# leeyevi/MV3D_TF

Measured on AMD Instinct MI355X. Metric: KITTI-shape frames/sec (RPN+3-view ROI-pool+NMS) at 1/2/4/8 MI355X, higher is better.
Workload: dtype f32; 1 GPU; BASELINE configs[2] path-only: batch 2, 3 views; proposal_layer_3d TRAIN cfg (23104 BEV anchors, pre/post-NMS 12000/2000, NMS 0.7) + anchor_target + proposal_target (256 sampled ROIs in batch 0) + FV ROIs + RoiPool 7x7 fwd+bwd on BEV 76x76x512 / RGB 46x155x512 / FV 8x64x512; peaky scores; driven by the library's own mv3d_train_path (submit -> counts to the host -> numpy-global-RNG draws on the hel; batch_per_gpu=2, ring_batches=16, streams=8, launch=path, hipgraph=False, parallelism=frames/1, pmc_signature=train/b2/r256/peaky/pair-tiles-planned

## Files before the change

include/mv3d_hip.h:

```cpp
#ifndef MV3D_HIP_H
#define MV3D_HIP_H
#include <stddef.h>
#include <stdint.h>
#ifdef __cplusplus
extern "C" {
#endif

typedef enum {
    MV3D_OK = 0,
    MV3D_ERR_INVALID_ARG = 1,
    MV3D_ERR_WORKSPACE = 2,
    MV3D_ERR_HIP = 3,
    MV3D_ERR_ZERO_DIVISION = 4
} mv3d_status;

int mv3d_version(void);
const char *mv3d_status_string(int status);


size_t mv3d_nms_workspace_bytes(int max_boxes);
int mv3d_nms_device(const float *dets_dev, int n, double thresh, int max_keep,
                    int32_t *keep_dev, int32_t *num_keep_dev, int32_t *status_dev,
                    void *workspace, size_t workspace_bytes, void *stream);

// ... 112 lines not shown
int mv3d_anchor_target_stage2(int H, int W, const mv3d_anchor_target_params *p,
                              const int32_t *disable_fg_dev, int n_dis_fg,
                              const int32_t *disable_bg1_dev, int n_dis_bg1,
                              const int32_t *disable_bg2_dev, int n_dis_bg2,
                              float *labels_dev, float *anchors_dev, float *anchors_3d_dev,
                              int32_t *n_anchors_dev, int anchors_cap,
                              void *workspace, size_t workspace_bytes, void *stream);

int mv3d_anchor_target_stage1_batch(int batch, int H, int W, const float *im_info_dev, const float *const *gt_bv_dev,
                                    const float *const *gt_3d_dev, const int *G, const mv3d_anchor_target_params *p,
                                    float *labels_dev, float *targets_dev, int32_t *const *counts_dev,
                                    uint8_t *const *fg_hi_dev, void *const *workspace, size_t workspace_bytes, void *stream);
int mv3d_anchor_target_stage1_batch_masked(int batch, int H, int W, const float *im_info_dev, const float *const *gt_bv_dev,
                                           const float *const *gt_3d_dev, const int *G, const mv3d_anchor_target_params *p,
                                           const uint8_t *const *anchor_mask_dev, float *labels_dev, float *targets_dev,
                                           int32_t *const *counts_dev, uint8_t *const *fg_hi_dev, void *const *workspace,
                                           size_t workspace_bytes, void *stream);
int mv3d_anchor_target_stage2_batch(int batch, int H, int W, const mv3d_anchor_target_params *p,
                                    const int32_t *const *disable_fg_dev, const int *n_dis_fg,
                                    const int32_t *const *disable_bg1_dev, const int *n_dis_bg1,
                                    const int32_t *const *disable_bg2_dev, const int *n_dis_bg2, float *labels_dev,
                                    float *anchors_dev, float *anchors_3d_dev, int32_t *n_anchors_dev, int anchors_cap,
                                    void *const *workspace, size_t workspace_bytes, void *stream);

typedef struct {
    int32_t num_classes;
    int32_t frame_index;
    double fg_thresh;
    double bg_thresh_hi;
    double bg_thresh_lo;
} mv3d_proposal_target_params;

size_t mv3d_proposal_target_workspace_bytes(int num_rois, int G);
int mv3d_proposal_target_stage1(const float *rois_bv_dev, const float *rois_3d_dev, int num_rois,
                                const float *gt_bv_dev, const float *gt_3d_dev, int G,
                                const mv3d_proposal_target_params *p, int32_t *counts_dev,
                                void *workspace, size_t workspace_bytes, void *stream);
int mv3d_proposal_target_stage2(const float *rois_bv_dev, const float *rois_3d_dev, int num_rois,
                                const float *gt_bv_dev, const float *gt_3d_dev,
                                const float *gt_corners_dev, int G, const float *calib_dev,
                                const mv3d_proposal_target_params *p,
                                const int32_t *fg_pick_dev, int n_fg, const int32_t *bg_pick_dev, int n_bg,
                                float *rois_bv_out, float *rois_img_out, int32_t *labels_out,
                                float *bbox_targets_out, float *rois_3d_out,
                                void *workspace, size_t workspace_bytes, void *stream);

// ... 13 lines not shown
                                           const int *num_rois_cap, const int32_t *const *num_rois_dev,
                                           const float *const *gt_bv_dev, const float *const *gt_3d_dev, const int *G,
                                           const mv3d_proposal_target_params *params, int32_t *const *counts_dev,
                                           void *const *workspace, const size_t *workspace_bytes, void *stream);
int mv3d_proposal_target_stage2_batch_devn(int batch, const float *const *rois_bv_dev, const float *const *rois_3d_dev,
                                           const int *num_rois_cap, const int32_t *const *num_rois_dev,
                                           const float *const *gt_bv_dev, const float *const *gt_3d_dev,
                                           const float *const *gt_corners_dev, const int *G, const float *const *calib_dev,
                                           const mv3d_proposal_target_params *params, const int32_t *const *fg_pick_dev,
                                           const int *n_fg, const int32_t *const *bg_pick_dev, const int *n_bg,
                                           float *const *rois_bv_out, float *const *rois_img_out, int32_t *const *labels_out,
                                           float *const *bbox_targets_out, float *const *rois_3d_out, float *const *rois_fv_out,
                                           void *const *workspace, const size_t *workspace_bytes, void *stream);

int mv3d_point_cloud_2_top(const float *points_dev, int num_points, float *top_dev, void *stream);

int mv3d_point_cloud_2_top_shape(double res, double zres, double side_lo, double side_hi, double fwd_lo, double fwd_hi,
                                 double height_lo, double height_hi, int *dims);
int mv3d_point_cloud_2_top_ranges(const float *points_dev, int num_points, double res, double zres, double side_lo, double side_hi,
                                  double fwd_lo, double fwd_hi, double height_lo, double height_hi, float *top_dev,
                                  int *status_dev, void *stream);

int mv3d_legacy_permutation(void *mt19937_state, int32_t n, int32_t *out);
typedef struct {
    int32_t n_fg, n_bg, n_low;
    int32_t pt_n_fg, pt_n_bg;
    int32_t reserved0;
    const uint8_t *fg_alive;
} mv3d_draw_frame;
typedef struct {
    int32_t rpn_batchsize;
    int32_t rpn_num_fg;
    int32_t rois_per_image;
    int32_t roi_fg_max;
} mv3d_draw_params;
int mv3d_draw_training_subsamples(void *mt19937_state, int batch, const mv3d_draw_frame *frames, const mv3d_draw_params *par,
                                  int32_t *lists, size_t lists_cap, int32_t *sizes, int32_t *scratch, size_t scratch_cap);

typedef struct {
    int32_t batch, H, W, num_classes;
    int32_t proposal_cap;
    int32_t anchor_cap;
    int32_t roi_cap;
    int32_t max_gt;
    mv3d_proposal_params proposal;
    mv3d_anchor_target_params anchor;
    mv3d_proposal_target_params target;
    mv3d_draw_params draw;
} mv3d_train_path_config;
typedef struct {
    float *blob_bv, *blob_img, *blob_3d;
    int32_t *num_proposals;
    void *proposal_ws; size_t proposal_ws_bytes;
    float *rpn_labels, *rpn_targets;
    float *anchors, *anchors_3d;
    int32_t *n_anchors;
    uint8_t *report; size_t report_row;
    int32_t *pt_counts;
    void *anchor_ws; size_t anchor_ws_bytes;
    void *target_ws; size_t target_ws_bytes;
// ... 237 lines not shown
```

mv3d_tf_amd/_lib.py:

```python
import ctypes as C
import os

import torch

_HERE = os.path.dirname(os.path.abspath(__file__))
LIB_PATH = os.path.join(_HERE, "libmv3d_hip.so")

OK, ERR_INVALID_ARG, ERR_WORKSPACE, ERR_HIP, ERR_ZERO_DIVISION = 0, 1, 2, 3, 4


class ProposalParams(C.Structure):
    _fields_ = [("feat_stride", C.c_int32), ("pre_nms_topN", C.c_int32), ("post_nms_topN", C.c_int32),
                ("img_height", C.c_int32), ("img_width", C.c_int32), ("img_padding", C.c_int32),
                ("nms_strict_gt", C.c_int32), ("reserved0", C.c_int32), ("nms_thresh", C.c_double), ("min_size", C.c_double)]


class DetectPostParams(C.Structure):
    _fields_ = [("num_classes", C.c_int32), ("rows_per_frame", C.c_int32), ("max_per_image", C.c_int32),
                ("nms_strict_gt", C.c_int32), ("score_thresh", C.c_float), ("reserved0", C.c_int32), ("nms_thresh", C.c_double)]


class AnchorTargetParams(C.Structure):
    _fields_ = [("feat_stride", C.c_int32), ("clobber_positives", C.c_int32),
                ("negative_overlap", C.c_double), ("positive_overlap", C.c_double)]
# ... 108 lines not shown
    "mv3d_proposal_3d_workspace_bytes": (C.c_size_t, [C.c_int, C.c_int, C.c_int, C.POINTER(ProposalParams)]),
    "mv3d_proposal_3d": (C.c_int, [_P, _P, C.c_int, C.c_int, C.c_int, _P, _P, C.POINTER(ProposalParams),
                                   _P, _P, _P, _P, _P, _P, C.c_size_t, _P]),
    "mv3d_proposal_3d_masked": (C.c_int, [_P, _P, C.c_int, C.c_int, C.c_int, _P, _P, C.POINTER(ProposalParams),
                                          _P, _P, _P, _P, _P, _P, _P, C.c_size_t, _P]),
    "mv3d_anchor_occupancy_workspace_bytes": (C.c_size_t, [C.c_int, C.c_int, C.c_int]),
    "mv3d_anchor_occupancy": (C.c_int, [_P, C.c_int, C.c_int, C.c_int, C.c_int, C.c_int, C.c_int, C.c_int, C.c_int, _P, _P, _P,
                                        C.c_size_t, _P]),
    "mv3d_roi_pool_forward": (C.c_int, [_P, C.c_float, C.c_int, C.c_int, C.c_int, C.c_int, C.c_int, C.c_int,
                                        C.c_int, _P, _P, _P, _P]),
    "mv3d_roi_pool_backward": (C.c_int, [_P, C.c_float, C.c_int, C.c_int, C.c_int, C.c_int, C.c_int, C.c_int,
                                         C.c_int, _P, _P, _P, _P]),
    "mv3d_anchor_target_workspace_bytes": (C.c_size_t, [C.c_int, C.c_int, C.c_int]),
    "mv3d_anchor_target_stage1": (C.c_int, [C.c_int, C.c_int, _P, _P, _P, C.c_int, C.POINTER(AnchorTargetParams),
                                            _P, _P, _P, _P, _P, C.c_size_t, _P]),
    "mv3d_anchor_target_stage2": (C.c_int, [C.c_int, C.c_int, C.POINTER(AnchorTargetParams), _P, C.c_int, _P,
                                            C.c_int, _P, C.c_int, _P, _P, _P, _P, C.c_int, _P, C.c_size_t, _P]),
    "mv3d_anchor_target_stage1_batch": (C.c_int, [C.c_int, C.c_int, C.c_int, _P, _P, _P, _P, C.POINTER(AnchorTargetParams), _P, _P, _P, _P,
                                                  _P, C.c_size_t, _P]),
    "mv3d_anchor_target_stage1_batch_masked": (C.c_int, [C.c_int, C.c_int, C.c_int, _P, _P, _P, _P, C.POINTER(AnchorTargetParams), _P, _P,
                                                         _P, _P, _P, _P, C.c_size_t, _P]),
    "mv3d_anchor_target_stage2_batch": (C.c_int, [C.c_int, C.c_int, C.c_int, C.POINTER(AnchorTargetParams), _P, _P, _P, _P, _P, _P, _P,
                                                  _P, _P, _P, C.c_int, _P, C.c_size_t, _P]),
    "mv3d_proposal_target_stage1_batch": (C.c_int, [C.c_int, _P, _P, _P, _P, _P, _P, _P, _P, _P, _P, _P]),
    "mv3d_proposal_target_stage2_batch": (C.c_int, [C.c_int, _P, _P, _P, _P, _P, _P, _P, _P, _P, _P, _P, _P, _P, _P, _P, _P, _P, _P, _P,
                                                    _P, _P, _P]),
    "mv3d_proposal_target_stage1_batch_devn": (C.c_int, [C.c_int, _P, _P, _P, _P, _P, _P, _P, _P, _P, _P, _P, _P]),
    "mv3d_proposal_target_stage2_batch_devn": (C.c_int, [C.c_int, _P, _P, _P, _P, _P, _P, _P, _P, _P, _P, _P, _P, _P, _P, _P, _P, _P, _P,
                                                         _P, _P, _P, _P, _P]),
    "mv3d_proposal_target_workspace_bytes": (C.c_size_t, [C.c_int, C.c_int]),
    "mv3d_proposal_target_stage1": (C.c_int, [_P, _P, C.c_int, _P, _P, C.c_int, C.POINTER(ProposalTargetParams), _P, _P,
                                              C.c_size_t, _P]),
    "mv3d_proposal_target_stage2": (C.c_int, [_P, _P, C.c_int, _P, _P, _P, C.c_int, _P, C.POINTER(ProposalTargetParams),
                                              _P, C.c_int, _P, C.c_int, _P, _P, _P, _P, _P, _P, C.c_size_t, _P]),
    "mv3d_point_cloud_2_top": (C.c_int, [_P, C.c_int, _P, _P]),
    "mv3d_point_cloud_2_top_shape": (C.c_int, [C.c_double] * 8 + [_P]),
    "mv3d_point_cloud_2_top_ranges": (C.c_int, [_P, C.c_int] + [C.c_double] * 8 + [_P, _P, _P]),
    "mv3d_box_detect_tail": (C.c_int, [_P, _P, C.c_int, C.c_int, _P, _P, _P, _P, _P]),
    "mv3d_detect_post_workspace_bytes": (C.c_size_t, [C.c_int, C.POINTER(DetectPostParams)]),
    "mv3d_detect_post": (C.c_int, [_P, _P, _P, _P, _P, C.c_int, C.POINTER(DetectPostParams), _P, _P, _P, _P, _P, _P, _P, C.c_size_t,
                                   _P]),
    "mv3d_detect_post_oriented_workspace_bytes": (C.c_size_t, [C.c_int, C.POINTER(DetectPostParams)]),
    "mv3d_detect_post_oriented": (C.c_int, [_P, _P, _P, _P, _P, C.c_int, C.POINTER(DetectPostParams), C.c_int, _P, _P, _P, _P, _P, _P,
                                            _P, C.c_size_t, _P]),
    "mv3d_loss_workspace_bytes": (C.c_size_t, [C.c_int]),
    "mv3d_rpn_loss": (C.c_int, [_P, _P, _P, _P, C.c_int, C.c_float, _P, _P, _P, _P, C.c_size_t, _P]),
    "mv3d_rcnn_loss": (C.c_int, [_P, _P, _P, _P, C.c_int, C.c_int, C.c_int, C.c_float, _P, _P, _P, _P, C.c_size_t, _P]),
    "mv3d_roi_pool_forward_views": (C.c_int, [C.c_int, C.POINTER(RoiView), C.c_int, C.c_int, _P]),
    "mv3d_roi_pool_forward_views_cold": (C.c_int, [C.c_int, C.POINTER(RoiView), C.c_int, C.c_int, _P]),
    "mv3d_roi_pool_forward_views_half": (C.c_int, [C.c_int, C.POINTER(RoiView), C.c_int, C.c_int, C.c_int, C.c_int, _P]),
    "mv3d_roi_pool_backward_workspace_bytes": (C.c_size_t, [C.c_int, C.POINTER(RoiGradView), C.c_int, C.c_int]),
    "mv3d_roi_pool_backward_views": (C.c_int, [C.c_int, C.POINTER(RoiGradView), C.c_int, C.c_int, _P, C.c_size_t, _P]),
    "mv3d_roi_pool_pair_workspace_bytes": (C.c_size_t, [C.c_int, C.POINTER(RoiGradView), C.c_int, C.c_int]),
    "mv3d_roi_pool_forward_views_pair": (C.c_int, [C.c_int, C.POINTER(RoiView), C.c_int, C.c_int, C.c_int, _P]),
    "mv3d_roi_pool_backward_views_pair": (C.c_int, [C.c_int, C.POINTER(RoiGradView), C.c_int, C.c_int, _P, C.c_size_t, _P]),
    "mv3d_roi_pool_argmax_decode": (C.c_int, [C.c_int, C.POINTER(RoiView), C.c_int, C.c_int, C.POINTER(C.c_void_p), _P]),
    "mv3d_ROIPoolForwardLaucher": (C.c_int, [_P, C.c_float, C.c_int, C.c_int, C.c_int, C.c_int, C.c_int, C.c_int, _P, _P, _P, _P]),
    "mv3d_ROIPoolBackwardLaucher": (C.c_int, [_P, C.c_float, C.c_int, C.c_int, C.c_int, C.c_int, C.c_int, C.c_int, C.c_int, _P, _P, _P, _P]),
    "mv3d_rois_3d_to_fv": (C.c_int, [_P, C.c_int, _P, _P]),
    "mv3d_legacy_permutation": (C.c_int, [_P, C.c_int32, _P]),
    "mv3d_draw_training_subsamples": (C.c_int, [_P, C.c_int, C.POINTER(DrawFrame), C.POINTER(DrawParams), _P, C.c_size_t, _P, _P,
                                                C.c_size_t]),
    "mv3d_train_path_create": (C.c_int, [C.POINTER(TrainPathConfig), C.c_int, C.POINTER(TrainPathSlot), C.c_int, C.POINTER(C.c_void_p)]),
    "mv3d_train_path_configure": (C.c_int, [_P, C.POINTER(TrainPathConfig)]),
    "mv3d_train_path_submit": (C.c_int, [_P, C.c_int, _P, _P, _P, _P, _P, _P, _P, _P, _P, _P]),
    "mv3d_train_path_submit_masked": (C.c_int, [_P, C.c_int, _P, _P, _P, _P, _P, _P, _P, _P, _P, _P, _P]),
    "mv3d_train_path_finish": (C.c_int, [_P, C.c_int, _P, _P, _P]),
    "mv3d_train_path_host_seconds": (C.c_int, [_P, C.POINTER(C.c_double), C.POINTER(C.c_double)]),
    "mv3d_train_path_destroy": (None, [_P]),
    "mv3d_gt_encode": (C.c_int, [_P, _P, C.c_int, _P, _P, _P, _P, _P, _P, _P]),
    "mv3d_conv3x3_f16": (C.c_int, [_P, _P, _P, _P, C.c_int, C.c_int, C.c_int, C.c_int, C.c_int, C.c_int, C.c_int, C.c_int, _P]),
    "mv3d_conv3x3_f32": (C.c_int, [_P, _P, _P, _P, C.c_int, C.c_int, C.c_int, C.c_int, C.c_int, C.c_int, C.c_int, _P]),
    "mv3d_maxpool2x2_f32": (C.c_int, [_P, _P, C.c_int, C.c_int, C.c_int, C.c_int, _P]),
    "mv3d_frame_nhwc_f32": (C.c_int, [_P, _P, C.c_int, C.c_int, C.c_int, C.c_int, C.c_int, _P]),
    "mv3d_conv3x3_bf16": (C.c_int, [_P, _P, _P, _P, C.c_int, C.c_int, C.c_int, C.c_int, C.c_int, C.c_int, C.c_int, C.c_int, _P]),
    "mv3d_maxpool2x2_bf16": (C.c_int, [_P, _P, C.c_int, C.c_int, C.c_int, C.c_int, _P]),
    "mv3d_frame_nhwc_bf16": (C.c_int, [_P, _P, C.c_int, C.c_int, C.c_int, C.c_int, C.c_int, _P]),
    "mv3d_conv3x3_wgrad_workspace_bytes": (C.c_size_t, [C.c_int, C.c_int, C.c_int, C.c_int, C.c_int]),
    "mv3d_conv3x3_wgrad_bf16": (C.c_int, [_P, _P, _P, _P, C.c_int, C.c_int, C.c_int, C.c_int, C.c_int, C.c_int, _P, C.c_size_t, _P]),
    "mv3d_conv3x3_wgrad_f32_workspace_bytes": (C.c_size_t, [C.c_int, C.c_int, C.c_int, C.c_int, C.c_int]),
    "mv3d_conv3x3_wgrad_f32": (C.c_int, [_P, _P, _P, _P, C.c_int, C.c_int, C.c_int, C.c_int, C.c_int, C.c_int, _P, C.c_size_t, _P]),
    "mv3d_conv3x3_pack_bf16": (C.c_int, [_P, _P, _P, C.c_int, C.c_int, C.c_int, _P]),
    "mv3d_conv3x3_gated_bf16": (C.c_int, [_P, _P, _P, _P, _P, C.c_int, C.c_int, C.c_int, C.c_int, C.c_int, _P]),
    "mv3d_maxpool2x2_bwd_f32": (C.c_int, [_P, _P, _P, C.c_int, C.c_int, C.c_int, C.c_int, _P]),
    "mv3d_maxpool2x2_bwd_bf16": (C.c_int, [_P, _P, _P, C.c_int, C.c_int, C.c_int, C.c_int, _P]),
# ... 70 lines not shown
```

mv3d_tf_amd/csrc/anchor_target.hip:

```cpp
#include <math.h>
#include "geometry.h"

__device__ __forceinline__ double mv3d_log(double x)
{
    if (x != x || x < 0) return NAN;
    if (x == 0) return -INFINITY;
    if (isinf(x)) return x;
    int k;
    double m = frexp(x, &k);
    if (m < 0.70710678118654752440) { m *= 2.0; k -= 1; }
    const double s = (m - 1.0) / (m + 1.0);
    const double z = s * s;
    double p = 1.0 / 39;
#pragma unroll
    for (int d = 37; d >= 1; d -= 2) p = fma(p, z, 1.0 / d);
    const double LN2_HI = 6.93147180369123816490e-01, LN2_LO = 1.90821492927058770002e-10;
    const double lm = 2.0 * s * p;
    return fma((double)k, LN2_HI, fma((double)k, LN2_LO, lm));
}

struct AtDev {
    int H, W, N, G, stride, clobber;
    double neg_ov, pos_ov;
    const float *im_info, *gt_bv, *gt_3d;
// ... 126 lines not shown
            f[0] = inside; f[1] = inside && (lab == 1.0f); f[2] = inside && (lab == 0.0f); f[3] = inside && (mx < neg_ov);
        },
        [&](int k, int pos, int n) {
            if (k == 1) { L.fg[pos] = n; fg_hi[pos] = (max_ov[n] >= neg_ov) ? 1 : 0; }
            else if (k == 2) L.bg[pos] = n;
            else if (k == 3) L.low[pos] = n;
        },
        F.agg1, tot);
    if (blockIdx.x == gridDim.x - 1 && threadIdx.x == 0) {
        int32_t *counts = F.counts;
        counts[0] = tot[0]; counts[1] = tot[1]; counts[2] = tot[2]; counts[3] = tot[3];
        counts[4] = counts[5] = counts[6] = counts[7] = 0;
    }
}

__global__ __launch_bounds__(256) void at_disable_all_kernel(AtBatch bt)
{
    const AtFrame &F = bt.f[blockIdx.y];
    const int n1 = F.n_dis_fg, n2 = F.n_dis_bg1, n3 = F.n_dis_bg2;
    for (int t = blockIdx.x * blockDim.x + threadIdx.x; t < n1 + n2 + n3; t += gridDim.x * blockDim.x) {
        if (t < n1) F.d.labels[F.lists.fg[F.dis_fg[t]]] = -1.0f;
        else if (t < n1 + n2) F.d.labels[F.lists.bg[F.dis_bg1[t - n1]]] = -1.0f;
        else F.d.argmax[F.lists.low[F.dis_bg2[t - n1 - n2]]] = -1;
    }
}

__global__ __launch_bounds__(256) void at_emit_relabel_kernel(AtBatch bt)
{
    const AtFrame &F = bt.f[blockIdx.y];
    const AtDev &d = F.d;
    float *anchors = F.anchors, *anchors_3d = F.anchors_3d;
    const int cap = bt.cap;
    int tot[1];
    mv3d_grid_compact<1>(
        d.N,
        [&](int n, bool f[1]) { f[0] = anchors && (d.max_ov[n] >= 0.0) && (d.labels[n] != -1.0f); },
        [&](int, int r, int n) {
            if (r >= cap) return;
            int x1, y1, x2, y2;
            grid_anchor(n, d.W, d.stride, x1, y1, x2, y2);
            float *A = anchors + 5 * (long long)r, *B = anchors_3d + 7 * (long long)r;
            A[0] = 0.0f; A[1] = (float)x1; A[2] = (float)y1; A[3] = (float)x2; A[4] = (float)y2;
            B[0] = 0.0f;
            anchor_to_lidar(x1, y1, x2, y2, B + 1);
        },
        F.agg2, tot);
// ... 85 lines not shown
    hipLaunchKernelGGL(at_compact_kernel, dim3(L.ncwg, batch), dim3(256), 0, s, bt);
    return mv3d_launch_status();
}

extern "C" int mv3d_anchor_target_stage1_batch(int batch, int H, int W, const float *im_info_dev, const float *const *gt_bv_dev,
                                               const float *const *gt_3d_dev, const int *G, const mv3d_anchor_target_params *p,
                                               float *labels_dev, float *targets_dev, int32_t *const *counts_dev,
                                               uint8_t *const *fg_hi_dev, void *const *workspace, size_t workspace_bytes,
                                               void *stream)
{
    return mv3d_anchor_target_stage1_batch_masked(batch, H, W, im_info_dev, gt_bv_dev, gt_3d_dev, G, p, nullptr, labels_dev, targets_dev,
                                                  counts_dev, fg_hi_dev, workspace, workspace_bytes, stream);
}

extern "C" int mv3d_anchor_target_stage1(int H, int W, const float *im_info_dev, const float *gt_bv_dev,
                                         const float *gt_3d_dev, int G, const mv3d_anchor_target_params *p,
                                         float *labels_dev, float *targets_dev, int32_t *counts_dev, uint8_t *fg_hi_dev,
                                         void *workspace, size_t workspace_bytes, void *stream)
{
    return mv3d_anchor_target_stage1_batch(1, H, W, im_info_dev, &gt_bv_dev, &gt_3d_dev, &G, p, labels_dev, targets_dev,
                                           &counts_dev, &fg_hi_dev, &workspace, workspace_bytes, stream);
}

extern "C" int mv3d_anchor_target_stage2_batch(int batch, int H, int W, const mv3d_anchor_target_params *p,
                                               const int32_t *const *disable_fg_dev, const int *n_dis_fg,
                                               const int32_t *const *disable_bg1_dev, const int *n_dis_bg1,
                                               const int32_t *const *disable_bg2_dev, const int *n_dis_bg2, float *labels_dev,
                                               float *anchors_dev, float *anchors_3d_dev, int32_t *n_anchors_dev,
                                               int anchors_cap, void *const *workspace, size_t workspace_bytes, void *stream)
{
    if (batch <= 0 || batch > AT_MAX_BATCH || !p || !labels_dev || !workspace || !n_dis_fg || !n_dis_bg1 || !n_dis_bg2 ||
        !disable_fg_dev || !disable_bg1_dev || !disable_bg2_dev)
        return MV3D_ERR_INVALID_ARG;
    AtLayout L;
    if (!at_layout(H, W, 0, L)) return MV3D_ERR_INVALID_ARG;
    const bool emit = anchors_dev && anchors_3d_dev && n_anchors_dev;
    AtBatch bt = {};
    bt.cap = anchors_cap;
    int most = 0;
    for (int b = 0; b < batch; ++b) {
        if (n_dis_fg[b] < 0 || n_dis_bg1[b] < 0 || n_dis_bg2[b] < 0) return MV3D_ERR_INVALID_ARG;
        if ((n_dis_fg[b] && !disable_fg_dev[b]) || (n_dis_bg1[b] && !disable_bg1_dev[b]) || (n_dis_bg2[b] && !disable_bg2_dev[b]))
            return MV3D_ERR_INVALID_ARG;
        if (!workspace[b] || workspace_bytes < L.total || ((uintptr_t)workspace[b] % MV3D_ALIGN)) return MV3D_ERR_WORKSPACE;
        AtFrame &F = bt.f[b];
        at_frame(F, L, H, W, 0, p, (char *)workspace[b]);
        F.d.im_info = nullptr; F.d.gt_bv = nullptr; F.d.gt_3d = nullptr; F.d.mask = nullptr; F.d.targets = nullptr;
        F.d.labels = labels_dev + (size_t)b * L.N;
        F.dis_fg = disable_fg_dev[b]; F.dis_bg1 = disable_bg1_dev[b]; F.dis_bg2 = disable_bg2_dev[b];
        F.n_dis_fg = n_dis_fg[b]; F.n_dis_bg1 = n_dis_bg1[b]; F.n_dis_bg2 = n_dis_bg2[b];
        F.anchors = emit ? anchors_dev + (size_t)b * anchors_cap * 5 : nullptr;
        F.anchors_3d = emit ? anchors_3d_dev + (size_t)b * anchors_cap * 7 : nullptr;
        F.n_anchors = emit ? n_anchors_dev + b : nullptr;
        const int n = n_dis_fg[b] + n_dis_bg1[b] + n_dis_bg2[b];
        if (n > most) most = n;
    }
    hipStream_t s = (hipStream_t)stream;
    if (most > 0) hipLaunchKernelGGL(at_disable_all_kernel, dim3((most + 255) / 256, batch), dim3(256), 0, s, bt);
    hipLaunchKernelGGL(at_emit_relabel_kernel, dim3(L.ncwg, batch), dim3(256), 0, s, bt);
    return mv3d_launch_status();
}

extern "C" int mv3d_anchor_target_stage2(int H, int W, const mv3d_anchor_target_params *p,
                                         const int32_t *disable_fg_dev, int n_dis_fg, const int32_t *disable_bg1_dev,
                                         int n_dis_bg1, const int32_t *disable_bg2_dev, int n_dis_bg2, float *labels_dev,
                                         float *anchors_dev, float *anchors_3d_dev, int32_t *n_anchors_dev,
                                         int anchors_cap, void *workspace, size_t workspace_bytes, void *stream)
{
    return mv3d_anchor_target_stage2_batch(1, H, W, p, &disable_fg_dev, &n_dis_fg, &disable_bg1_dev, &n_dis_bg1, &disable_bg2_dev,
                                           &n_dis_bg2, labels_dev, anchors_dev, anchors_3d_dev, n_anchors_dev, anchors_cap,
                                           &workspace, workspace_bytes, stream);
}
```

mv3d_tf_amd/csrc/legacy_rng.hip:

```cpp
#include <stdint.h>
#include <string.h>
#include "../../include/mv3d_hip.h"

namespace {

constexpr int MT_N = 624, MT_M = 397;
struct MtState { uint32_t key[MT_N]; int pos; };

inline void mt_gen(MtState *s)
{
    uint32_t *k = s->key;
    int i;
    for (i = 0; i < MT_N - MT_M; ++i) {
        const uint32_t y = (k[i] & 0x80000000u) | (k[i + 1] & 0x7fffffffu);
        k[i] = k[i + MT_M] ^ (y >> 1) ^ ((y & 1u) ? 0x9908b0dfu : 0u);
    }
    for (; i < MT_N - 1; ++i) {
        const uint32_t y = (k[i] & 0x80000000u) | (k[i + 1] & 0x7fffffffu);
        k[i] = k[i + (MT_M - MT_N)] ^ (y >> 1) ^ ((y & 1u) ? 0x9908b0dfu : 0u);
    }
    const uint32_t y = (k[MT_N - 1] & 0x80000000u) | (k[0] & 0x7fffffffu);
    k[MT_N - 1] = k[MT_M - 1] ^ (y >> 1) ^ ((y & 1u) ? 0x9908b0dfu : 0u);
    s->pos = 0;
}
// ... 25 lines not shown
                for (int k = pos; k < MT_N; ++k) {
                    uint32_t y = s->key[k];
                    y ^= (y >> 11);
                    y ^= (y << 7) & 0x9d2c5680u;
                    y ^= (y << 15) & 0xefc60000u;
                    y ^= (y >> 18);
                    t[k] = y;
                }
                t_lo = pos;
            }
            while (pos < MT_N && i > lo) {
                const uint32_t j = t[pos++] & mask;
                const bool ok = j <= (uint32_t)i;
                const uint32_t jj = ok ? j : (uint32_t)i;
                const int32_t a = x[i], b = x[jj];
                x[i] = b; x[jj] = a;
                i -= ok ? 1 : 0;
            }
        }
    }
    s->pos = pos;
}

}

extern "C" int mv3d_legacy_permutation(void *mt19937_state, int32_t n, int32_t *out)
{
    if (!mt19937_state || n < 0 || (n > 0 && !out)) return MV3D_ERR_INVALID_ARG;
    MtState *s = (MtState *)mt19937_state;
    if (s->pos < 0 || s->pos > MT_N) return MV3D_ERR_INVALID_ARG;
    permutation(s, n, out);
    return MV3D_OK;
}

extern "C" int mv3d_draw_training_subsamples(void *mt19937_state, int batch, const mv3d_draw_frame *frames,
                                             const mv3d_draw_params *par, int32_t *lists, size_t lists_cap, int32_t *sizes,
                                             int32_t *scratch, size_t scratch_cap)
{
    if (!mt19937_state || batch <= 0 || !frames || !par || !lists || !sizes || !scratch) return MV3D_ERR_INVALID_ARG;
    MtState *s = (MtState *)mt19937_state;
    if (s->pos < 0 || s->pos > MT_N) return MV3D_ERR_INVALID_ARG;
    size_t o = 0;
    auto emit = [&](int32_t n, int32_t take, bool draw, int32_t *size_out) -> bool {
        *size_out = 0;
        if (!draw) return true;
        if (n < 0 || (size_t)n > scratch_cap || take < 0 || take > n || o + (size_t)take > lists_cap) return false;
// ... 15 lines not shown
        const int32_t num_fg = par->rpn_num_fg;
        const int32_t *dis_fg = lists + o;
        if (!emit(f.n_fg, f.n_fg - num_fg, f.n_fg > num_fg, &sz[0])) return MV3D_ERR_WORKSPACE;
        const int32_t num_bg = par->rpn_batchsize - (f.n_fg < num_fg ? f.n_fg : num_fg);
        if (!emit(f.n_bg, f.n_bg - num_bg, f.n_bg > num_bg, &sz[1])) return MV3D_ERR_WORKSPACE;
        int32_t n_pos = 0;
        if (f.n_fg > 0) {
            if ((size_t)f.n_fg > scratch_cap) return MV3D_ERR_WORKSPACE;
            uint8_t *alive = (uint8_t *)scratch;
            for (int32_t i = 0; i < f.n_fg; ++i) alive[i] = f.fg_alive[i] ? 1 : 0;
            for (int32_t i = 0; i < sz[0]; ++i) alive[dis_fg[i]] = 0;
            for (int32_t i = 0; i < f.n_fg; ++i) n_pos += alive[i];
        }
        const int32_t num_bg2 = par->rpn_batchsize - n_pos;
        if (!emit(f.n_low, f.n_low - num_bg2, f.n_low > num_bg2, &sz[2])) return MV3D_ERR_WORKSPACE;
        const int32_t fg_n = par->roi_fg_max < f.pt_n_fg ? par->roi_fg_max : f.pt_n_fg;
        if (!emit(f.pt_n_fg, fg_n, f.pt_n_fg > 0, &sz[3])) return MV3D_ERR_WORKSPACE;
        const int32_t bg_room = par->rois_per_image - fg_n;
        const int32_t bg_n = bg_room < f.pt_n_bg ? bg_room : f.pt_n_bg;
        if (!emit(f.pt_n_bg, bg_n < 0 ? 0 : bg_n, f.pt_n_bg > 0, &sz[4])) return MV3D_ERR_WORKSPACE;
    }
    return MV3D_OK;
}
```

mv3d_tf_amd/csrc/train_stream.hip:

```cpp
#include <hip/hip_runtime.h>
#include <chrono>
#include <condition_variable>
#include <deque>
#include <mutex>
#include <new>
#include <thread>
#include <vector>
#include "common.h"
#include "../../include/mv3d_hip.h"

#define TP_MAX_BATCH 16

namespace {

enum SlotState { TP_IDLE = 0, TP_SUBMITTED = 1, TP_STAGED = 2 };

struct Slot {
    mv3d_train_path_slot buf;
    hipEvent_t ev = nullptr;
    int state = TP_IDLE, rc = MV3D_OK;
    hipStream_t stream = nullptr;
    void *mt = nullptr;
    const float *calib = nullptr;
    const float *gt_bv[TP_MAX_BATCH], *gt_3d[TP_MAX_BATCH], *gt_c[TP_MAX_BATCH];
    int G[TP_MAX_BATCH];
    int32_t sizes[5 * TP_MAX_BATCH], rows[TP_MAX_BATCH];
    std::vector<uint8_t> spill[TP_MAX_BATCH];
    float *p_bv[TP_MAX_BATCH], *p_3d[TP_MAX_BATCH];
    int32_t *p_num[TP_MAX_BATCH], *p_cnt[TP_MAX_BATCH], *a_cnt[TP_MAX_BATCH];
    uint8_t *a_fgh[TP_MAX_BATCH];
    void *a_ws[TP_MAX_BATCH], *p_ws[TP_MAX_BATCH];
    int p_cap[TP_MAX_BATCH];
    size_t p_wsz[TP_MAX_BATCH];
    uint8_t *dv_report = nullptr;
    int32_t *dv_pt_counts = nullptr, *dv_num_proposals = nullptr;
};

static bool tp_force_copies()
{
#ifdef MV3D_TUNING
    return getenv("MV3D_TRAIN_PATH_COPIES") != nullptr;
#else
    return false;
#endif
}

__global__ __launch_bounds__(256) void tp_report_kernel(const uint8_t *__restrict__ report, size_t report_row, uint8_t *__restrict__ h_report,
                                                        size_t h_row, int B, const int32_t *__restrict__ pt_counts, int32_t *__restrict__ h_pt,
                                                        const int32_t *__restrict__ nump, int32_t *__restrict__ h_nump)
{
    const size_t v = h_row / 16;
    for (size_t i = threadIdx.x; i < (size_t)B * v; i += 256) {
        const size_t b = i / v, j = i - b * v;
        reinterpret_cast<uint4 *>(h_report + b * h_row)[j] = reinterpret_cast<const uint4 *>(report + b * report_row)[j];
    }
    for (int i = threadIdx.x; i < 4 * B; i += 256) h_pt[i] = pt_counts[i];
    for (int i = threadIdx.x; i < 2 * B; i += 256) h_nump[i] = nump[i];
}
// ... 75 lines not shown
    const int B = c.batch, H = c.H, W = c.W;
    const auto t0 = std::chrono::steady_clock::now();
    TP_HIP(hipEventSynchronize(s.ev));
    const auto t1 = std::chrono::steady_clock::now();
    for (int b = 0; b < B; ++b)
        if (u.h_num_proposals[B + b] & MV3D_FLAG_ZERO_DIVISION) return MV3D_ERR_ZERO_DIVISION;
    mv3d_draw_frame fr[TP_MAX_BATCH];
    for (int b = 0; b < B; ++b) {
        const uint8_t *head = u.h_report + (size_t)b * u.h_report_row;
        const int32_t *cnt = (const int32_t *)head;
        fr[b].n_fg = cnt[1]; fr[b].n_bg = cnt[2]; fr[b].n_low = cnt[3];
        fr[b].pt_n_fg = u.h_pt_counts[4 * b + 1]; fr[b].pt_n_bg = u.h_pt_counts[4 * b + 2];
        fr[b].reserved0 = 0;
        if (cnt[1] < 0 || (size_t)cnt[1] > (size_t)4 * H * W) return MV3D_ERR_INVALID_ARG;
        if (32 + (size_t)cnt[1] <= u.h_report_row) {
            fr[b].fg_alive = head + 32;
        } else {
            s.spill[b].resize((size_t)cnt[1]);
            TP_HIP(hipMemcpyAsync(s.spill[b].data(), s.a_fgh[b], (size_t)cnt[1], hipMemcpyDeviceToHost, s.stream));
            TP_HIP(hipStreamSynchronize(s.stream));
            fr[b].fg_alive = s.spill[b].data();
        }
    }
    int rc = mv3d_draw_training_subsamples(s.mt, B, fr, &c.draw, u.h_lists, u.lists_cap, s.sizes, u.h_scratch, u.scratch_cap);
    const auto t2 = std::chrono::steady_clock::now();
    {
        std::lock_guard<std::mutex> g(tp->m);
        tp->t_wait += std::chrono::duration<double>(t1 - t0).count();
        tp->t_draw += std::chrono::duration<double>(t2 - t1).count();
    }
    if (rc != MV3D_OK) return rc;
    size_t off[5 * TP_MAX_BATCH + 1];
    off[0] = 0;
    for (int k = 0; k < 5 * B; ++k) off[k + 1] = off[k] + (size_t)s.sizes[k];
    const int32_t *const lists = u.lists;
    if (off[5 * B]) TP_HIP(hipMemcpyAsync(u.lists, u.h_lists, off[5 * B] * sizeof(int32_t), hipMemcpyHostToDevice, s.stream));
    const int32_t *lst[5][TP_MAX_BATCH];
    int cnt[5][TP_MAX_BATCH];
    for (int b = 0; b < B; ++b)
        for (int k = 0; k < 5; ++k) {
            cnt[k][b] = s.sizes[5 * b + k];
            lst[k][b] = cnt[k][b] ? lists + off[5 * b + k] : nullptr;
        }
    rc = mv3d_anchor_target_stage2_batch(B, H, W, &c.anchor, lst[0], cnt[0], lst[1], cnt[1], lst[2], cnt[2], u.rpn_labels, u.anchors,
                                         u.anchors_3d, u.n_anchors, c.anchor_cap, s.a_ws, u.anchor_ws_bytes, s.stream);
    if (rc != MV3D_OK) return rc;
    float *o_bev[TP_MAX_BATCH], *o_rgb[TP_MAX_BATCH], *o_fv[TP_MAX_BATCH], *o_3d[TP_MAX_BATCH], *o_tg[TP_MAX_BATCH];
    int32_t *o_lab[TP_MAX_BATCH];
    const float *cal[TP_MAX_BATCH];
    size_t row = 0;
    for (int b = 0; b < B; ++b) {
        const int S = cnt[3][b] + cnt[4][b];
        s.rows[b] = S;
        if (row + (size_t)S > (size_t)B * c.roi_cap) return MV3D_ERR_WORKSPACE;
        o_bev[b] = S ? u.rois_bev + row * 5 : nullptr;
        o_rgb[b] = S ? u.rois_rgb + row * 5 : nullptr;
        o_fv[b] = (S && u.rois_fv) ? u.rois_fv + row * 5 : nullptr;
        o_3d[b] = S ? u.rois_3d + row * 7 : nullptr;
        o_lab[b] = S ? u.labels + row : nullptr;
        o_tg[b] = S ? u.bbox_targets + row * 24 * c.num_classes : nullptr;
        cal[b] = s.calib + (size_t)b * 48;
        row += (size_t)S;
    }
    return mv3d_proposal_target_stage2_batch_devn(B, s.p_bv, s.p_3d, s.p_cap, s.p_num, s.gt_bv, s.gt_3d, s.gt_c, s.G, cal, tp->tpar, lst[3],
                                                  cnt[3], lst[4], cnt[4], o_bev, o_rgb, o_lab, o_tg, o_3d, u.rois_fv ? o_fv : nullptr, s.p_ws,
                                                  s.p_wsz, s.stream);
}

// ... 40 lines not shown
    mv3d_train_path *tp = new (std::nothrow) mv3d_train_path();
    if (!tp) return MV3D_ERR_HIP;
    set_params(tp, *config);
    tp->depth = depth;
    if (hipGetDevice(&tp->device) != hipSuccess) { delete tp; return MV3D_ERR_HIP; }
    try {
        tp->slots.resize((size_t)depth);
    } catch (...) {
        delete tp;
        return MV3D_ERR_HIP;
    }
    for (int k = 0; k < depth; ++k) {
        Slot &s = tp->slots[k];
        s.buf = slots[k];
        slot_tables(tp->cfg, s);
        {
            void *d0 = nullptr, *d1 = nullptr, *d2 = nullptr;
            const bool mapped = hipHostGetDevicePointer(&d0, s.buf.h_report, 0) == hipSuccess && hipHostGetDevicePointer(&d1, s.buf.h_pt_counts, 0) == hipSuccess &&
                                hipHostGetDevicePointer(&d2, s.buf.h_num_proposals, 0) == hipSuccess && d0 && d1 && d2;
            (void)hipGetLastError();
            if (mapped && s.buf.h_report_row % 16 == 0 && (uintptr_t)d0 % 16 == 0 && (uintptr_t)s.buf.report % 16 == 0 && !tp_force_copies()) {
                s.dv_report = (uint8_t *)d0; s.dv_pt_counts = (int32_t *)d1; s.dv_num_proposals = (int32_t *)d2;
            }
        }
        if (hipEventCreateWithFlags(&s.ev, hipEventDisableTiming | hipEventBlockingSync) != hipSuccess) {
            for (int j = 0; j < k; ++j) (void)hipEventDestroy(tp->slots[j].ev);
            delete tp;
            return MV3D_ERR_HIP;
        }
    }
    tp->threaded = helper_thread != 0;
    if (tp->threaded) {
        try {
            tp->helper = std::thread(helper_main, tp);
        } catch (...) {
            for (Slot &s : tp->slots) (void)hipEventDestroy(s.ev);
            delete tp;
            return MV3D_ERR_HIP;
        }
    }
    *out = tp;
    return MV3D_OK;
}

extern "C" int mv3d_train_path_configure(mv3d_train_path *tp, const mv3d_train_path_config *c)
{
// ... 134 lines not shown
```

Measured before the change: 16670 frames/s.

## Draw only kept tail of RNG permutations and pass keep-bitmasks to anchor disable

Host-side subsampling now computes only the last k entries of the legacy MT19937 permutation. It uses a sparse swap map and an SSE block-skip over the rejection-sampled prefix, so it no longer builds the full n-element shuffle for large candidate sets. Those entries are encoded as per-frame keep bitmasks instead of explicit disable index lists. A new disable kernel reads the bitmasks. The lists buffer is read through a mapped host pointer when available, which skips the H2D copy. This adds complex RNG-equivalence logic that must reproduce numpy's stream exactly, and zero-copy reads from pinned host memory over the bus.

```diff
diff --git a/include/mv3d_hip.h b/include/mv3d_hip.h
--- a/include/mv3d_hip.h
+++ b/include/mv3d_hip.h
@@ -158,6 +158,12 @@
                                     const int32_t *const *disable_bg2_dev, const int *n_dis_bg2, float *labels_dev,
                                     float *anchors_dev, float *anchors_3d_dev, int32_t *n_anchors_dev, int anchors_cap,
                                     void *const *workspace, size_t workspace_bytes, void *stream);
+int mv3d_anchor_target_stage2_batch_kept(int batch, int H, int W, const mv3d_anchor_target_params *p,
+                                         const int32_t *const *keep_fg_dev, const int *n_fg,
+                                         const int32_t *const *keep_bg1_dev, const int *n_bg,
+                                         const int32_t *const *keep_bg2_dev, const int *n_low, float *labels_dev,
+                                         float *anchors_dev, float *anchors_3d_dev, int32_t *n_anchors_dev, int anchors_cap,
+                                         void *const *workspace, size_t workspace_bytes, void *stream);
 
 typedef struct {
     int32_t num_classes;
@@ -217,6 +223,7 @@
                                   int *status_dev, void *stream);
 
 int mv3d_legacy_permutation(void *mt19937_state, int32_t n, int32_t *out);
+int mv3d_legacy_permutation_tail(void *mt19937_state, int32_t n, int32_t k, int32_t *out);
 typedef struct {
     int32_t n_fg, n_bg, n_low;
     int32_t pt_n_fg, pt_n_bg;
@@ -231,6 +238,8 @@
 } mv3d_draw_params;
 int mv3d_draw_training_subsamples(void *mt19937_state, int batch, const mv3d_draw_frame *frames, const mv3d_draw_params *par,
                                   int32_t *lists, size_t lists_cap, int32_t *sizes, int32_t *scratch, size_t scratch_cap);
+int mv3d_draw_training_subsamples_kept(void *mt19937_state, int batch, const mv3d_draw_frame *frames, const mv3d_draw_params *par,
+                                       int32_t *lists, size_t lists_cap, int32_t *sizes, int32_t *scratch, size_t scratch_cap);
 
 typedef struct {
     int32_t batch, H, W, num_classes;
diff --git a/mv3d_tf_amd/_lib.py b/mv3d_tf_amd/_lib.py
--- a/mv3d_tf_amd/_lib.py
+++ b/mv3d_tf_amd/_lib.py
@@ -154,6 +154,8 @@
                                                          _P, _P, _P, _P, C.c_size_t, _P]),
     "mv3d_anchor_target_stage2_batch": (C.c_int, [C.c_int, C.c_int, C.c_int, C.POINTER(AnchorTargetParams), _P, _P, _P, _P, _P, _P, _P,
                                                   _P, _P, _P, C.c_int, _P, C.c_size_t, _P]),
+    "mv3d_anchor_target_stage2_batch_kept": (C.c_int, [C.c_int, C.c_int, C.c_int, C.POINTER(AnchorTargetParams), _P, _P, _P, _P, _P, _P,
+                                                       _P, _P, _P, _P, C.c_int, _P, C.c_size_t, _P]),
     "mv3d_proposal_target_stage1_batch": (C.c_int, [C.c_int, _P, _P, _P, _P, _P, _P, _P, _P, _P, _P, _P]),
     "mv3d_proposal_target_stage2_batch": (C.c_int, [C.c_int, _P, _P, _P, _P, _P, _P, _P, _P, _P, _P, _P, _P, _P, _P, _P, _P, _P, _P, _P,
                                                     _P, _P, _P]),
@@ -193,6 +195,9 @@
     "mv3d_legacy_permutation": (C.c_int, [_P, C.c_int32, _P]),
     "mv3d_draw_training_subsamples": (C.c_int, [_P, C.c_int, C.POINTER(DrawFrame), C.POINTER(DrawParams), _P, C.c_size_t, _P, _P,
                                                 C.c_size_t]),
+    "mv3d_legacy_permutation_tail": (C.c_int, [_P, C.c_int32, C.c_int32, _P]),
+    "mv3d_draw_training_subsamples_kept": (C.c_int, [_P, C.c_int, C.POINTER(DrawFrame), C.POINTER(DrawParams), _P, C.c_size_t, _P, _P,
+                                                     C.c_size_t]),
     "mv3d_train_path_create": (C.c_int, [C.POINTER(TrainPathConfig), C.c_int, C.POINTER(TrainPathSlot), C.c_int, C.POINTER(C.c_void_p)]),
     "mv3d_train_path_configure": (C.c_int, [_P, C.POINTER(TrainPathConfig)]),
     "mv3d_train_path_submit": (C.c_int, [_P, C.c_int, _P, _P, _P, _P, _P, _P, _P, _P, _P, _P]),
diff --git a/mv3d_tf_amd/csrc/anchor_target.hip b/mv3d_tf_amd/csrc/anchor_target.hip
--- a/mv3d_tf_amd/csrc/anchor_target.hip
+++ b/mv3d_tf_amd/csrc/anchor_target.hip
@@ -172,6 +172,27 @@
         if (t < n1) F.d.labels[F.lists.fg[F.dis_fg[t]]] = -1.0f;
         else if (t < n1 + n2) F.d.labels[F.lists.bg[F.dis_bg1[t - n1]]] = -1.0f;
         else F.d.argmax[F.lists.low[F.dis_bg2[t - n1 - n2]]] = -1;
+    }
+}
+
+__global__ __launch_bounds__(256) void at_disable_kept_kernel(AtBatch bt)
+{
+    const AtFrame &F = bt.f[blockIdx.y];
+    const int n1 = F.n_dis_fg, n2 = F.n_dis_bg1, n3 = F.n_dis_bg2;
+    const unsigned N = (unsigned)F.d.N;
+    for (int t = blockIdx.x * blockDim.x + threadIdx.x; t < n1 + n2 + n3; t += gridDim.x * blockDim.x) {
+        if (t < n1) {
+            const unsigned a = (unsigned)F.lists.fg[t];
+            if (!((F.dis_fg[t >> 5] >> (t & 31)) & 1) && a < N) F.d.labels[a] = -1.0f;
+        } else if (t < n1 + n2) {
+            const int u = t - n1;
+            const unsigned a = (unsigned)F.lists.bg[u];
+            if (!((F.dis_bg1[u >> 5] >> (u & 31)) & 1) && a < N) F.d.labels[a] = -1.0f;
+        } else {
+            const int u = t - n1 - n2;
+            const unsigned a = (unsigned)F.lists.low[u];
+            if (!((F.dis_bg2[u >> 5] >> (u & 31)) & 1) && a < N) F.d.argmax[a] = -1;
+        }
     }
 }
 
@@ -303,12 +324,11 @@
                                            &counts_dev, &fg_hi_dev, &workspace, workspace_bytes, stream);
 }
 
-extern "C" int mv3d_anchor_target_stage2_batch(int batch, int H, int W, const mv3d_anchor_target_params *p,
-                                               const int32_t *const *disable_fg_dev, const int *n_dis_fg,
-                                               const int32_t *const *disable_bg1_dev, const int *n_dis_bg1,
-                                               const int32_t *const *disable_bg2_dev, const int *n_dis_bg2, float *labels_dev,
-                                               float *anchors_dev, float *anchors_3d_dev, int32_t *n_anchors_dev,
-                                               int anchors_cap, void *const *workspace, size_t workspace_bytes, void *stream)
+static int at_stage2(bool kept, int batch, int H, int W, const mv3d_anchor_target_params *p, const int32_t *const *disable_fg_dev,
+                     const int *n_dis_fg, const int32_t *const *disable_bg1_dev, const int *n_dis_bg1,
+                     const int32_t *const *disable_bg2_dev, const int *n_dis_bg2, float *labels_dev, float *anchors_dev,
+                     float *anchors_3d_dev, int32_t *n_anchors_dev, int anchors_cap, void *const *workspace, size_t workspace_bytes,
+                     void *stream)
 {
     if (batch <= 0 || batch > AT_MAX_BATCH || !p || !labels_dev || !workspace || !n_dis_fg || !n_dis_bg1 || !n_dis_bg2 ||
         !disable_fg_dev || !disable_bg1_dev || !disable_bg2_dev)
@@ -323,6 +343,7 @@
         if (n_dis_fg[b] < 0 || n_dis_bg1[b] < 0 || n_dis_bg2[b] < 0) return MV3D_ERR_INVALID_ARG;
         if ((n_dis_fg[b] && !disable_fg_dev[b]) || (n_dis_bg1[b] && !disable_bg1_dev[b]) || (n_dis_bg2[b] && !disable_bg2_dev[b]))
             return MV3D_ERR_INVALID_ARG;
+        if (kept && (n_dis_fg[b] > L.N || n_dis_bg1[b] > L.N || n_dis_bg2[b] > L.N)) return MV3D_ERR_INVALID_ARG;
         if (!workspace[b] || workspace_bytes < L.total || ((uintptr_t)workspace[b] % MV3D_ALIGN)) return MV3D_ERR_WORKSPACE;
         AtFrame &F = bt.f[b];
         at_frame(F, L, H, W, 0, p, (char *)workspace[b]);
@@ -337,9 +358,32 @@
         if (n > most) most = n;
     }
     hipStream_t s = (hipStream_t)stream;
-    if (most > 0) hipLaunchKernelGGL(at_disable_all_kernel, dim3((most + 255) / 256, batch), dim3(256), 0, s, bt);
+    if (most > 0 && kept) hipLaunchKernelGGL(at_disable_kept_kernel, dim3((most + 255) / 256, batch), dim3(256), 0, s, bt);
+    else if (most > 0) hipLaunchKernelGGL(at_disable_all_kernel, dim3((most + 255) / 256, batch), dim3(256), 0, s, bt);
     hipLaunchKernelGGL(at_emit_relabel_kernel, dim3(L.ncwg, batch), dim3(256), 0, s, bt);
     return mv3d_launch_status();
+}
+
+extern "C" int mv3d_anchor_target_stage2_batch(int batch, int H, int W, const mv3d_anchor_target_params *p,
+                                               const int32_t *const *disable_fg_dev, const int *n_dis_fg,
+                                               const int32_t *const *disable_bg1_dev, const int *n_dis_bg1,
+                                               const int32_t *const *disable_bg2_dev, const int *n_dis_bg2, float *labels_dev,
+                                               float *anchors_dev, float *anchors_3d_dev, int32_t *n_anchors_dev,
+                                               int anchors_cap, void *const *workspace, size_t workspace_bytes, void *stream)
+{
+    return at_stage2(false, batch, H, W, p, disable_fg_dev, n_dis_fg, disable_bg1_dev, n_dis_bg1, disable_bg2_dev, n_dis_bg2, labels_dev,
+                     anchors_dev, anchors_3d_dev, n_anchors_dev, anchors_cap, workspace, workspace_bytes, stream);
+}
+
+extern "C" int mv3d_anchor_target_stage2_batch_kept(int batch, int H, int W, const mv3d_anchor_target_params *p,
+                                                    const int32_t *const *keep_fg_dev, const int *n_fg,
+                                                    const int32_t *const *keep_bg1_dev, const int *n_bg,
+                                                    const int32_t *const *keep_bg2_dev, const int *n_low, float *labels_dev,
+                                                    float *anchors_dev, float *anchors_3d_dev, int32_t *n_anchors_dev,
+                                                    int anchors_cap, void *const *workspace, size_t workspace_bytes, void *stream)
+{
+    return at_stage2(true, batch, H, W, p, keep_fg_dev, n_fg, keep_bg1_dev, n_bg, keep_bg2_dev, n_low, labels_dev, anchors_dev,
+                     anchors_3d_dev, n_anchors_dev, anchors_cap, workspace, workspace_bytes, stream);
 }
 
 extern "C" int mv3d_anchor_target_stage2(int H, int W, const mv3d_anchor_target_params *p,
diff --git a/mv3d_tf_amd/csrc/legacy_rng.hip b/mv3d_tf_amd/csrc/legacy_rng.hip
--- a/mv3d_tf_amd/csrc/legacy_rng.hip
+++ b/mv3d_tf_amd/csrc/legacy_rng.hip
@@ -1,5 +1,9 @@
 #include <stdint.h>
+#include <stdlib.h>
 #include <string.h>
+#if defined(__SSE2__)
+#include <emmintrin.h>
+#endif
 #include "../../include/mv3d_hip.h"
 
 namespace {
@@ -71,6 +75,142 @@
     s->pos = pos;
 }
 
+constexpr int32_t TAIL_MAX_KEPT = 1024;
+constexpr int TAIL_TABLE = 4 * TAIL_MAX_KEPT;
+
+inline bool tail_falls_back(int32_t n, int32_t k) { return k > TAIL_MAX_KEPT || (int64_t)4 * k > n; }
+
+struct SparseMap {
+    int32_t key[TAIL_TABLE], val[TAIL_TABLE];
+    uint32_t bits, msk;
+    explicit SparseMap(int32_t k)
+    {
+        bits = 4;
+        while ((int32_t)(1u << bits) < 4 * k) ++bits;
+        msk = (1u << bits) - 1u;
+        for (uint32_t h = 0; h <= msk; ++h) key[h] = -1;
+    }
+    int32_t *at(int32_t j)
+    {
+        uint32_t h = ((uint32_t)j * 2654435761u) >> (32 - bits);
+        while (key[h] != -1 && key[h] != j) h = (h + 1) & msk;
+        if (key[h] == -1) { key[h] = j; val[h] = j; }
+        return &val[h];
+    }
+};
+
+#if defined(__SSE2__)
+inline int scan_blocks(const uint32_t *t, int pos, uint32_t mask, int32_t lo, int32_t &i)
+{
+    const __m128i vmask = _mm_set1_epi32((int32_t)mask), v16 = _mm_set1_epi32(16);
+    __m128i vi = _mm_set1_epi32(i);
+    for (; pos + 16 <= MT_N; pos += 16) {
+        int32_t is = _mm_cvtsi128_si32(vi);
+        if (is - 16 < lo) break;
+        const __m128i vsure = _mm_sub_epi32(vi, v16);
+        __m128i unsure = _mm_setzero_si128(), between = _mm_setzero_si128();
+        for (int q = 0; q < 16; q += 4) {
+            const __m128i m = _mm_and_si128(_mm_loadu_si128((const __m128i *)(t + pos + q)), vmask);
+            const __m128i gs = _mm_cmpgt_epi32(m, vsure), gi = _mm_cmpgt_epi32(m, vi);
+            unsure = _mm_add_epi32(unsure, gs);
+            between = _mm_or_si128(between, _mm_xor_si128(gs, gi));
+        }
+        if (_mm_movemask_epi8(between)) {
+            for (int q = 0; q < 16; ++q) is -= ((int32_t)(t[pos + q] & mask) <= is) ? 1 : 0;
+            vi = _mm_set1_epi32(is);
+            continue;
+        }
+        unsure = _mm_add_epi32(unsure, _mm_shuffle_epi32(unsure, 0x4E));
+        unsure = _mm_add_epi32(unsure, _mm_shuffle_epi32(unsure, 0xB1));
+        vi = _mm_sub_epi32(vi, _mm_add_epi32(v16, unsure));
+    }
+    i = _mm_cvtsi128_si32(vi);
+    return pos;
+}
+#else
+inline int scan_blocks(const uint32_t *t, int pos, uint32_t mask, int32_t lo, int32_t &i)
+{
+    for (; pos + 16 <= MT_N && i - 16 >= lo; pos += 16) {
+        int32_t sure = 0, maybe = 0;
+        for (int q = 0; q < 16; ++q) {
+            const int32_t m = (int32_t)(t[pos + q] & mask);
+            sure += (m <= i - 16) ? 1 : 0;
+            maybe += (m <= i) ? 1 : 0;
+        }
+        if (maybe == sure) { i -= sure; continue; }
+        for (int q = 0; q < 16; ++q) i -= ((int32_t)(t[pos + q] & mask) <= i) ? 1 : 0;
+    }
+    return pos;
+}
+#endif
+
+void permutation_tail(MtState *s, int32_t n, int32_t k, int32_t *out, int32_t *scratch)
+{
+    if (n <= 1) {
+        if (k == 1) out[0] = 0;
+        return;
+    }
+    if (tail_falls_back(n, k)) {
+        permutation(s, n, scratch);
+        memcpy(out, scratch + (n - k), (size_t)k * sizeof(int32_t));
+        return;
+    }
+    const int32_t base = n - k;
+    for (int32_t q = 0; q < k; ++q) out[q] = base + q;
+    SparseMap below(k);
+    int32_t i = n - 1;
+    int pos = s->pos;
+    uint32_t t[MT_N];
+    int t_lo = MT_N;
+    while (i >= 1) {
+        const uint32_t mask = 0xffffffffu >> __builtin_clz((uint32_t)i);
+        const int32_t lo = (int32_t)(mask >> 1);
+        while (i > lo) {
+            if (pos == MT_N) { mt_gen(s); pos = 0; t_lo = MT_N; }
+            if (t_lo > pos) {
+                for (int q = pos; q < MT_N; ++q) {
+                    uint32_t y = s->key[q];
+                    y ^= (y >> 11);
+                    y ^= (y << 7) & 0x9d2c5680u;
+                    y ^= (y << 15) & 0xefc60000u;
+                    y ^= (y >> 18);
+                    t[q] = y;
+                }
+                t_lo = pos;
+            }
+            if (i >= base) {
+                while (pos < MT_N && i > lo && i >= base) {
+                    const int32_t j = (int32_t)(t[pos++] & mask);
+                    if (j > i) continue;
+                    int32_t *pi = out + (i - base), *pj = j >= base ? out + (j - base) : below.at(j);
+                    const int32_t a = *pi;
+                    *pi = *pj; *pj = a;
+                    --i;
+                }
+            } else {
+                pos = scan_blocks(t, pos, mask, lo, i);
+                while (pos < MT_N && i > lo) i -= ((int32_t)(t[pos++] & mask) <= i) ? 1 : 0;
+            }
+        }
+    }
+    s->pos = pos;
+}
+
+}
+
+extern "C" int mv3d_legacy_permutation_tail(void *mt19937_state, int32_t n, int32_t k, int32_t *out)
+{
+    if (!mt19937_state || n < 0 || k < 0 || k > n || (k > 0 && !out)) return MV3D_ERR_INVALID_ARG;
+    MtState *s = (MtState *)mt19937_state;
+    if (s->pos < 0 || s->pos > MT_N) return MV3D_ERR_INVALID_ARG;
+    int32_t *scratch = nullptr;
+    if (n > 1 && tail_falls_back(n, k)) {
+        scratch = (int32_t *)malloc((size_t)n * sizeof(int32_t));
+        if (!scratch) return MV3D_ERR_WORKSPACE;
+    }
+    permutation_tail(s, n, k, out, scratch);
+    free(scratch);
+    return MV3D_OK;
 }
 
 extern "C" int mv3d_legacy_permutation(void *mt19937_state, int32_t n, int32_t *out)
@@ -132,3 +272,74 @@
     }
     return MV3D_OK;
 }
+
+extern "C" int mv3d_draw_training_subsamples_kept(void *mt19937_state, int batch, const mv3d_draw_frame *frames,
+                                                  const mv3d_draw_params *par, int32_t *lists, size_t lists_cap, int32_t *sizes,
+                                                  int32_t *scratch, size_t scratch_cap)
+{
+    if (!mt19937_state || batch <= 0 || !frames || !par || !lists || !sizes || !scratch) return MV3D_ERR_INVALID_ARG;
+    MtState *s = (MtState *)mt19937_state;
+    if (s->pos < 0 || s->pos > MT_N) return MV3D_ERR_INVALID_ARG;
+    size_t o = 0;
+    int32_t kept_buf[TAIL_MAX_KEPT];
+    auto emit_kept = [&](int32_t n, int32_t take, bool draw, int32_t *size_out) -> bool {
+        *size_out = 0;
+        if (!draw) return true;
+        const size_t words = ((size_t)(n > 0 ? n : 0) + 31) / 32;
+        if (n < 0 || (size_t)n > scratch_cap || take < 0 || take > n || o + words > lists_cap) return false;
+        const int32_t k = n - take;
+        const int32_t *kept = kept_buf;
+        if (k <= TAIL_MAX_KEPT) {
+            permutation_tail(s, n, k, kept_buf, scratch);
+        } else {
+            permutation(s, n, scratch);
+            kept = scratch + take;
+        }
+        uint32_t *bits = (uint32_t *)(lists + o);
+        memset(bits, 0, words * sizeof(uint32_t));
+        for (int32_t q = 0; q < k; ++q) bits[kept[q] >> 5] |= 1u << (kept[q] & 31);
+        *size_out = take;
+        o += words;
+        return true;
+    };
+    auto emit = [&](int32_t n, int32_t take, bool draw, int32_t *size_out) -> bool {
+        *size_out = 0;
+        if (!draw) return true;
+        if (n < 0 || (size_t)n > scratch_cap || take < 0 || take > n || o + (size_t)take > lists_cap) return false;
+        if (take == n) {
+            permutation(s, n, lists + o);
+        } else {
+            permutation(s, n, scratch);
+            memcpy(lists + o, scratch, (size_t)take * sizeof(int32_t));
+        }
+        *size_out = take;
+        o += (size_t)take;
+        return true;
+    };
+    for (int b = 0; b < batch; ++b) {
+        const mv3d_draw_frame &f = frames[b];
+        int32_t *sz = sizes + 5 * b;
+        if (f.n_fg < 0 || f.n_bg < 0 || f.n_low < 0 || f.pt_n_fg < 0 || f.pt_n_bg < 0 || (f.n_fg > 0 && !f.fg_alive))
+            return MV3D_ERR_INVALID_ARG;
+        const int32_t num_fg = par->rpn_num_fg;
+        const uint32_t *keep_fg = (const uint32_t *)(lists + o);
+        if (!emit_kept(f.n_fg, f.n_fg - num_fg, f.n_fg > num_fg, &sz[0])) return MV3D_ERR_WORKSPACE;
+        const int32_t num_bg = par->rpn_batchsize - (f.n_fg < num_fg ? f.n_fg : num_fg);
+        if (!emit_kept(f.n_bg, f.n_bg - num_bg, f.n_bg > num_bg, &sz[1])) return MV3D_ERR_WORKSPACE;
+        int32_t n_pos = 0;
+        if (f.n_fg > 0) {
+            if ((size_t)f.n_fg > scratch_cap) return MV3D_ERR_WORKSPACE;
+            const bool drawn = sz[0] > 0;
+            for (int32_t i = 0; i < f.n_fg; ++i)
+                n_pos += (f.fg_alive[i] && (!drawn || ((keep_fg[i >> 5] >> (i & 31)) & 1u))) ? 1 : 0;
+        }
+        const int32_t num_bg2 = par->rpn_batchsize - n_pos;
+        if (!emit_kept(f.n_low, f.n_low - num_bg2, f.n_low > num_bg2, &sz[2])) return MV3D_ERR_WORKSPACE;
+        const int32_t fg_n = par->roi_fg_max < f.pt_n_fg ? par->roi_fg_max : f.pt_n_fg;
+        if (!emit(f.pt_n_fg, fg_n, f.pt_n_fg > 0, &sz[3])) return MV3D_ERR_WORKSPACE;
+        const int32_t bg_room = par->rois_per_image - fg_n;
+        const int32_t bg_n = bg_room < f.pt_n_bg ? bg_room : f.pt_n_bg;
+        if (!emit(f.pt_n_bg, bg_n < 0 ? 0 : bg_n, f.pt_n_bg > 0, &sz[4])) return MV3D_ERR_WORKSPACE;
+    }
+    return MV3D_OK;
+}
diff --git a/mv3d_tf_amd/csrc/train_stream.hip b/mv3d_tf_amd/csrc/train_stream.hip
--- a/mv3d_tf_amd/csrc/train_stream.hip
+++ b/mv3d_tf_amd/csrc/train_stream.hip
@@ -34,6 +34,7 @@
     size_t p_wsz[TP_MAX_BATCH];
     uint8_t *dv_report = nullptr;
     int32_t *dv_pt_counts = nullptr, *dv_num_proposals = nullptr;
+    const int32_t *dv_lists = nullptr;
 };
 
 static bool tp_force_copies()
@@ -155,7 +156,7 @@
             fr[b].fg_alive = s.spill[b].data();
         }
     }
-    int rc = mv3d_draw_training_subsamples(s.mt, B, fr, &c.draw, u.h_lists, u.lists_cap, s.sizes, u.h_scratch, u.scratch_cap);
+    int rc = mv3d_draw_training_subsamples_kept(s.mt, B, fr, &c.draw, u.h_lists, u.lists_cap, s.sizes, u.h_scratch, u.scratch_cap);
     const auto t2 = std::chrono::steady_clock::now();
     {
         std::lock_guard<std::mutex> g(tp->m);
@@ -163,20 +164,25 @@
         tp->t_draw += std::chrono::duration<double>(t2 - t1).count();
     }
     if (rc != MV3D_OK) return rc;
+    int cnt[5][TP_MAX_BATCH];
     size_t off[5 * TP_MAX_BATCH + 1];
     off[0] = 0;
-    for (int k = 0; k < 5 * B; ++k) off[k + 1] = off[k] + (size_t)s.sizes[k];
-    const int32_t *const lists = u.lists;
-    if (off[5 * B]) TP_HIP(hipMemcpyAsync(u.lists, u.h_lists, off[5 * B] * sizeof(int32_t), hipMemcpyHostToDevice, s.stream));
+    for (int b = 0; b < B; ++b) {
+        const int32_t n_cand[3] = {fr[b].n_fg, fr[b].n_bg, fr[b].n_low};
+        for (int k = 0; k < 5; ++k) {
+            const int32_t sz = s.sizes[5 * b + k];
+            cnt[k][b] = k < 3 ? (sz > 0 ? n_cand[k] : 0) : sz;
+            off[5 * b + k + 1] = off[5 * b + k] + (size_t)(k < 3 ? (cnt[k][b] + 31) / 32 : sz);
+        }
+    }
+    const int32_t *const lists = s.dv_lists ? s.dv_lists : u.lists;
+    if (!s.dv_lists && off[5 * B])
+        TP_HIP(hipMemcpyAsync(u.lists, u.h_lists, off[5 * B] * sizeof(int32_t), hipMemcpyHostToDevice, s.stream));
     const int32_t *lst[5][TP_MAX_BATCH];
-    int cnt[5][TP_MAX_BATCH];
     for (int b = 0; b < B; ++b)
-        for (int k = 0; k < 5; ++k) {
-            cnt[k][b] = s.sizes[5 * b + k];
-            lst[k][b] = cnt[k][b] ? lists + off[5 * b + k] : nullptr;
-        }
-    rc = mv3d_anchor_target_stage2_batch(B, H, W, &c.anchor, lst[0], cnt[0], lst[1], cnt[1], lst[2], cnt[2], u.rpn_labels, u.anchors,
-                                         u.anchors_3d, u.n_anchors, c.anchor_cap, s.a_ws, u.anchor_ws_bytes, s.stream);
+        for (int k = 0; k < 5; ++k) lst[k][b] = cnt[k][b] ? lists + off[5 * b + k] : nullptr;
+    rc = mv3d_anchor_target_stage2_batch_kept(B, H, W, &c.anchor, lst[0], cnt[0], lst[1], cnt[1], lst[2], cnt[2], u.rpn_labels, u.anchors,
+                                              u.anchors_3d, u.n_anchors, c.anchor_cap, s.a_ws, u.anchor_ws_bytes, s.stream);
     if (rc != MV3D_OK) return rc;
     float *o_bev[TP_MAX_BATCH], *o_rgb[TP_MAX_BATCH], *o_fv[TP_MAX_BATCH], *o_3d[TP_MAX_BATCH], *o_tg[TP_MAX_BATCH];
     int32_t *o_lab[TP_MAX_BATCH];
@@ -263,6 +269,10 @@
             if (mapped && s.buf.h_report_row % 16 == 0 && (uintptr_t)d0 % 16 == 0 && (uintptr_t)s.buf.report % 16 == 0 && !tp_force_copies()) {
                 s.dv_report = (uint8_t *)d0; s.dv_pt_counts = (int32_t *)d1; s.dv_num_proposals = (int32_t *)d2;
             }
+            void *d3 = nullptr;
+            if (hipHostGetDevicePointer(&d3, s.buf.h_lists, 0) == hipSuccess && d3 && (uintptr_t)d3 % 4 == 0 && !tp_force_copies())
+                s.dv_lists = (const int32_t *)d3;
+            (void)hipGetLastError();
         }
         if (hipEventCreateWithFlags(&s.ev, hipEventDisableTiming | hipEventBlockingSync) != hipSuccess) {
             for (int j = 0; j < k; ++j) (void)hipEventDestroy(tp->slots[j].ev);
```

Result: no change. 16670 frames/s, median of 2 (-0.0%).
